# shubhamchandak94/Spring

Hardware: AMD Instinct MI355X
Metric: Mreads/s through reorder stage (higher is better)
Workload: dtype u64

## Files before the change

spring_amd/csrc/reorder_device.h:

```cpp
#ifndef SPRING_REORDER_DEVICE_H_
#define SPRING_REORDER_DEVICE_H_

#include <hip/hip_runtime.h>
#include <stdint.h>

namespace sr {

constexpr int MAX_READ_LEN = 511;
constexpr int MAX_SEARCH = 1000;
constexpr int THRESH = 4;
constexpr uint32_t DEEP_BIN = 16;
constexpr uint32_t MID_BIN = 64;
constexpr uint32_t BIG_BIN = 256;
constexpr uint32_t CHUNK = 64;
constexpr uint32_t MARK_BLOCK = 256;
constexpr uint32_t MC_WAVES_PER_BLOCK = MARK_BLOCK / 4 + 3;
constexpr int UBLK_SHIFT = 12;
constexpr int LDS_PAD = 10;
constexpr int LDS_LIMBS = 16 + 2 * LDS_PAD;

enum { MODE_SEARCH = 0, MODE_NEED_SEED = 1 };
enum { PROP_NONE = 0, PROP_MATCH = 1, PROP_SEED = 2, PROP_FRESH = 3  };
enum { PK_NONE = 0, PK_MATCH = 1, PK_SEED = 2, PK_NOSEED = 4, PK_DONE = 5 };
constexpr unsigned long long PK_CURSOR_BIT = 1ull << 35;
// ... 35 lines not shown
  uint64_t st_probes, st_keyok, st_cands, st_iter, st_lost, st_hits, n_unmatched, st_long ;
#ifdef SR_PHASE_TIMING
  uint64_t pt[64];
#endif
};
#ifndef SR_PHASE_TIMING
static_assert(sizeof(Chain) == 384, "Chain layout");
#endif

struct Globals {
  long long cursor;
  uint32_t alive;
  uint32_t e_alloc;
  uint32_t s_alloc;
  uint32_t pad;
  long long cursor_b;
};

struct TabView {
  const uint4 *buck;
  int bshift;
  int minz;
  int lshift;
};
constexpr uint32_t TAG_MARK = 0xfffffffcu;
constexpr int MINZ_HEAVY = 12;
constexpr int MINZ_K = 16;
constexpr int MINZ_WL = 32;

constexpr int LONG_MAX_BINS = 1024;
constexpr int LONG_MAX_PARTS = 64;
struct LongHead {
  uint32_t nb, nparts, best_single, bestrid;
  uint32_t bestpart, pad[3];
  uint32_t blo[LONG_MAX_PARTS + 4];
  uint32_t rescode[LONG_MAX_PARTS], resrid[LONG_MAX_PARTS];
  uint32_t capped[LONG_MAX_PARTS];
};
struct DevParams {
  const uint64_t *reads;
  const uint16_t *lens;
  uint32_t n;
  int L, W, S, Lpad, maxshift, uniform_len;
  int plan[2][6];
  int seed_wide;
  int deep_bins;
// ... 43 lines not shown
  unsigned long long *prop;
  uint32_t *alive_wave;
  Chain *chains;
  int4 *cnt;
  uint32_t *cnt8;
  uint4 *e_rec; uint2 *e_chunk;
  uint32_t *s_rec; uint2 *s_chunk;
  uint32_t *f_order; char *f_rc; char *f_flag; long long *f_pos; uint16_t *f_len; uint32_t *f_order_s;
};

void launch_unpack(hipStream_t st, const uint8_t *dna, const uint64_t *off, uint32_t n, int L, int W, int S,
                   uint32_t rec_fixed, uint64_t *reads, uint16_t *lens, uint32_t *bad_len = nullptr);
void launch_flag_in_dict(hipStream_t st, const uint16_t *lens, uint32_t n, int dend, uint32_t *flag);
void launch_keys(hipStream_t st, const uint64_t *reads, const uint16_t *lens, const uint32_t *slot, uint32_t n,
                 int S, int dstart, int dend, uint64_t *keys, uint32_t *vals);
struct DictBuild {
  const uint32_t *ustart, *ucount, *ids;
  ulonglong2 *urec;
  uint32_t *deep, *ndeep;
};
void launch_tab_insert(hipStream_t st, const uint64_t *mhash, const uint64_t *mval, uint64_t nmerged, DictBuild d0,
                       DictBuild d1, uint32_t *fpt, int bshift);
void launch_minz_prepare(hipStream_t st, const uint64_t *mhash, const uint64_t *mval, uint64_t nmerged, DictBuild d0,
                         DictBuild d1, int lshift, uint32_t *bucket, uint64_t *tagpay);
void launch_tab_insert_minz(hipStream_t st, const uint32_t *bucket_sorted, const uint64_t *tagpay_sorted, uint64_t nmerged,
                            uint32_t *fpt, int bshift, uint32_t *marked);
hipError_t sort_pairs_u32_u64(hipStream_t st, void *tmp, size_t &tmp_bytes, const uint32_t *kin, uint32_t *kout,
                              const uint64_t *vin, uint64_t *vout, size_t n, unsigned end_bit);
hipError_t merge_by_hash(hipStream_t st, void *tmp, size_t &tmp_bytes, const uint64_t *k0, const uint64_t *k1,
                         const uint64_t *v0, const uint64_t *v1, uint64_t *kout, uint64_t *vout, size_t n0, size_t n1);
void launch_iota_tag(hipStream_t st, uint64_t *v, uint64_t n, uint64_t tag);
void launch_build_epos(hipStream_t st, const uint32_t *ids, uint64_t m, uint32_t *epos);
void launch_trim_bins(hipStream_t st, const uint32_t *deep, const uint32_t *ndeep, uint32_t ndeep_host,
                      ulonglong2 *urec, const uint32_t *ids, const uint64_t *taken, ulonglong2 *sig ,
                      uint32_t *epos = nullptr );
void launch_build_sig(hipStream_t st, const uint32_t *ids, uint64_t m, const uint64_t *reads, int S, int W, ulonglong2 *sig);
void launch_dict_lookup(hipStream_t st, TabView tab, const ulonglong2 *urec, int which,
                        const uint64_t *reads, int S, int dstart, int dend, const uint64_t *keys, uint32_t nkeys,
                        uint32_t *start, uint32_t *count);
void launch_fill_u32(hipStream_t st, uint32_t *p, uint64_t n, uint32_t v);
void launch_init_taken(hipStream_t st, uint64_t *taken, uint64_t nwords, uint32_t n, uint32_t *ublk);
void launch_init_chains(hipStream_t st, const DevParams &P, bool seeds = true);
void launch_check_seed_state(hipStream_t st, const DevParams &P, uint64_t nwords, unsigned long long *bad);
void launch_search(hipStream_t st, const DevParams &P, bool stats);
void launch_apply(hipStream_t st, const DevParams &P, bool literal);
void launch_round(hipStream_t st, const DevParams &P, bool stats, bool mg);
void launch_mg_resolve(hipStream_t st, const DevParams &P);
void launch_mg_mark(hipStream_t st, const DevParams &P);
void launch_ph_mark(hipStream_t st, const DevParams &P);
// ... 33 lines not shown
```

spring_amd/csrc/reorder_kernels.hip:

```cpp
#include <cstdlib>
#include <cstring>
#include <hip/hip_runtime.h>
#include <rocprim/rocprim.hpp>

#include "reorder_device.h"
#include "synth_common.h"

namespace sr {


__device__ __forceinline__ uint64_t mix64(uint64_t x) {
  x ^= x >> 33; x *= 0xff51afd7ed558ccdull; x ^= x >> 33; x *= 0xc4ceb9fe1a85ec53ull; x ^= x >> 33;
  return x;
}

__device__ __forceinline__ void wave_sync() {
  __builtin_amdgcn_fence(__ATOMIC_SEQ_CST, "wavefront");
  __builtin_amdgcn_wave_barrier();
}

__device__ __forceinline__ int uni_i32(int v) { return __builtin_amdgcn_readfirstlane(v); }
template <class T>
__device__ __forceinline__ T *uni_ptr(T *p) {
  const uint64_t a = reinterpret_cast<uint64_t>(p);
// ... 55 lines not shown
  return f == 0u ? 1u : f == 0x3fffffffu ? 0x3ffffffeu : f;
}
__device__ __forceinline__ uint64_t bucket_of(uint64_t h, int bshift) { return h >> bshift; }
__device__ __forceinline__ uint64_t bucket_mask(int bshift) { return (1ull << (64 - bshift)) - 1; }
__device__ __forceinline__ uint64_t unmix64(uint64_t x) {
  x ^= x >> 33; x *= 0x9cb4b2f8129337dbull; x ^= x >> 33; x *= 0x4f74430c22a54005ull; x ^= x >> 33;
  return x;
}
__device__ __forceinline__ uint32_t fmix32(uint32_t x) {
  x ^= x >> 16; x *= 0x85ebca6bu; x ^= x >> 13; x *= 0xc2b2ae35u; x ^= x >> 16;
  return x;
}
__device__ __forceinline__ uint32_t kmer_order(uint32_t x) {
  uint32_t r = __builtin_bitreverse32(x);
  r = ~(((r >> 1) & 0x55555555u) | ((r & 0x55555555u) << 1));
  return ((x < r ? x : r) ^ 0x5bd1e995u) * 0x9e3779b1u;
}
__device__ __forceinline__ uint32_t minz_of_key(uint64_t key) {
  uint32_t m = 0xffffffffu;
#pragma unroll
  for (int q = 0; q <= MINZ_WL - MINZ_K; q++) m = min(m, kmer_order((uint32_t)(key >> (2 * q))));
  return fmix32(m);
}
__device__ __forceinline__ uint64_t tab_home(const TabView &T, uint64_t h, uint32_t mz) {
  return T.minz ? (((uint64_t)(mz >> T.lshift) << 2) | ((h >> 30) & 3ull)) : bucket_of(h, T.bshift);
}
__device__ __forceinline__ uint64_t tab_redirect_x(uint32_t x32, int bshift) { return mix64(0x6a09e667f3bcc908ull ^ x32) >> bshift; }
__device__ __forceinline__ uint64_t tab_redirect(const TabView &T, uint64_t h) {
  return tab_redirect_x(fp30_of(h) | ((uint32_t)((h >> 30) & 3ull) << 30), T.bshift);
}
template <bool MZ = false>
__device__ __forceinline__ int tab_find(const TabView &T, uint64_t h, uint32_t mz, int l, int skip,
                                        uint32_t &pay, bool &other) {
  const uint32_t mine = (fp30_of(h) << 2) | ((uint32_t)l << 1), theirs = mine ^ 2u;
  const uint64_t bmask = bucket_mask(T.bshift);
  uint64_t b = MZ ? tab_home(T, h, mz) : bucket_of(h, T.bshift);
  bool first = MZ && T.minz != 0;
  for (;;) {
#if defined(SR_TAGS_NT)
    typedef uint32_t u32x4_t __attribute__((ext_vector_type(4)));
    const u32x4_t tv = __builtin_nontemporal_load(reinterpret_cast<const u32x4_t *>(&T.buck[b * 2]));
    const uint4 t = make_uint4(tv.x, tv.y, tv.z, tv.w);
#elif defined(SR_TAGS_SC)
    typedef uint32_t u32x4_t __attribute__((ext_vector_type(4)));
    u32x4_t tv;
    asm volatile("global_load_dwordx4 %0, %1, off sc0 sc1\n\ts_waitcnt vmcnt(0)" : "=v"(tv) : "v"(&T.buck[b * 2]) : "memory");
    const uint4 t = make_uint4(tv.x, tv.y, tv.z, tv.w);
#else
    const uint4 t = T.buck[b * 2];
#endif
    if (MZ && first) {
      first = false;
      if (t.x == TAG_MARK) { b = tab_redirect(T, h); continue; }
    }
    other = other || (t.x & ~1u) == theirs || (t.y & ~1u) == theirs || (t.z & ~1u) == theirs || t.w != 0;
    uint32_t m = (uint32_t)((t.x & ~1u) == mine) | ((uint32_t)((t.y & ~1u) == mine) << 1) |
                 ((uint32_t)((t.z & ~1u) == mine) << 2) | ((uint32_t)((t.w & ~1u) == mine) << 3);
    const int c = __popc(m);
    if (c > skip) {
// ... 111 lines not shown
  if (cn >= BIG_BIN) atomicAdd(d.ndeep + 1, cn);
  if (cn >= MID_BIN) atomicAdd(d.ndeep + 2, cn);
  d.urec[u] = make_ulonglong2(unmix64(h), (uint64_t)st | ((uint64_t)cn << 32));
  if (!OVERFLOW) {
    fpt[b0 * 8 + rank] = tag;
    fpt[b0 * 8 + 4 + rank] = pay;
    return;
  }
  const uint64_t bmask = bucket_mask(bshift);
  uint64_t b = (b0 + 1) & bmask;
  for (;;) {
    uint32_t *bk = fpt + b * 8;
    for (int sl = 0; sl < 4; sl++) {
      if (atomicCAS(bk + sl, 0u, tag) == 0u) {
        bk[4 + sl] = pay;
        return;
      }
    }
    b = (b + 1) & bmask;
  }
}

__global__ void k_minz_prepare(const uint64_t *__restrict__ mhash, const uint64_t *__restrict__ mval, uint64_t nm,
                               DictBuild d0, DictBuild d1, int lshift, uint32_t *__restrict__ bucket,
                               uint64_t *__restrict__ tagpay) {
  const uint64_t i = (uint64_t)blockIdx.x * blockDim.x + threadIdx.x;
  if (i >= nm) return;
  const uint64_t h = mhash[i], key = unmix64(h);
  const uint64_t mv = mval[i];
  const uint32_t l = (uint32_t)(mv >> 63), u = (uint32_t)mv;
  const DictBuild &d = l ? d1 : d0;
  const uint32_t st = d.ustart[u], cn = d.ucount[u];
  const bool single = cn == 1;
  const uint32_t tag = (fp30_of(h) << 2) | (l << 1) | (single ? 1u : 0u);
  const uint32_t pay = single ? d.ids[st] : u;
  if (cn >= DEEP_BIN) d.deep[atomicAdd(d.ndeep, 1u)] = u;
  if (cn >= BIG_BIN) atomicAdd(d.ndeep + 1, cn);
  if (cn >= MID_BIN) atomicAdd(d.ndeep + 2, cn);
  d.urec[u] = make_ulonglong2(key, (uint64_t)st | ((uint64_t)cn << 32));
  bucket[i] = ((minz_of_key(key) >> lshift) << 2) | (uint32_t)((h >> 30) & 3ull);
  tagpay[i] = (uint64_t)tag | ((uint64_t)pay << 32);
}
template <bool SECOND>
__global__ void k_tab_insert_minz(const uint32_t *__restrict__ bk, const uint64_t *__restrict__ tp, uint64_t nm,
                                  uint32_t *fpt, int bshift, uint32_t *marked ) {
  const uint64_t i = (uint64_t)blockIdx.x * blockDim.x + threadIdx.x;
  if (i >= nm) return;
  const uint32_t b0 = bk[i], line = b0 >> 2;
  int back = 0;
  while (back <= MINZ_HEAVY && i > (uint64_t)back && (bk[i - 1 - back] >> 2) == line) back++;
  bool heavy = back > MINZ_HEAVY;
  if (!heavy) {
    const uint64_t at = i - back + MINZ_HEAVY;
    heavy = at < nm && (bk[at] >> 2) == line;
  }
  int rank = 0;
  if (!heavy) while (rank < 4 && rank < back && bk[i - 1 - rank] == b0) rank++;
  const uint64_t w = tp[i];
  const uint32_t tag = (uint32_t)w, pay = (uint32_t)(w >> 32);
  if (!SECOND) {
    if (heavy) {
      if (back == 0) {
        for (int s = 0; s < 4; s++) fpt[((uint64_t)line * 4 + s) * 8] = TAG_MARK;
        atomicAdd(marked, 1u);
      }
    } else if (rank < 4) {
      fpt[(uint64_t)b0 * 8 + rank] = tag;
      fpt[(uint64_t)b0 * 8 + 4 + rank] = pay;
    }
    return;
  }
  if (!heavy && rank < 4) return;
  const uint64_t bmask = bucket_mask(bshift);
  uint64_t b = heavy ? tab_redirect_x((tag >> 2) | ((b0 & 3u) << 30), bshift) : (((uint64_t)b0 + 1) & bmask);
  for (;;) {
// ... 33 lines not shown
    const uint32_t pos = w + (uint32_t)__popcll(m & ((1ull << lane) - 1));
    if (live && pos != j) {
      ids[start + pos] = r;
      if (sig) sig[start + pos] = sg;
      if (epos) epos[r] = start + pos;
    }
    w += (uint32_t)__popcll(m);
  }
  if (lane == 0 && w != count) urec[u].y = (uint64_t)start | ((uint64_t)w << 32);
}

__global__ void k_dict_lookup(TabView tab, const ulonglong2 *__restrict__ urec, int which,
                              const uint64_t *__restrict__ reads, int S, int dstart, int klen2,
                              const uint64_t *__restrict__ keys, uint32_t nkeys, uint32_t *__restrict__ start,
                              uint32_t *__restrict__ count) {
  uint32_t i = blockIdx.x * blockDim.x + threadIdx.x;
  if (i >= nkeys) return;
  const uint64_t key = keys[i], h = mix64(key);
  const uint32_t mz = tab.minz ? minz_of_key(key) : 0u;
  uint32_t s = 0, c = 0xffffffffu;
  for (int skip = 0;; skip++) {
    uint32_t pay;
    bool other = false;
    const int kind = tab_find<true>(tab, h, mz, which, skip, pay, other);
    if (kind == 0) break;
    if (kind == 1) {
      const ulonglong2 r = urec[pay];
      if (r.x != key) continue;
      s = (uint32_t)r.y; c = (uint32_t)(r.y >> 32);
      break;
    }
    if (read_window(reads + (uint64_t)pay * S, S, dstart, klen2) != key) continue;
    s = pay; c = 1u | 0x80000000u;
    break;
  }
  start[i] = s;
  count[i] = c;
}

__global__ void k_fill_u32(uint32_t *p, uint64_t n, uint32_t v) {
  uint64_t i = (uint64_t)blockIdx.x * blockDim.x + threadIdx.x;
  if (i < n) p[i] = v;
}

__global__ void k_init_taken(uint64_t *taken, uint64_t nwords, uint32_t n, uint32_t *ublk) {
  uint64_t w = (uint64_t)blockIdx.x * blockDim.x + threadIdx.x;
  if (w >= nwords) return;
// ... 508 lines not shown
                                           bool &keyok, uint32_t &ncand, bool &other, lds_u32_t *s_best, lds_u32_t *stage,
                                           int lane, PendBin *pend = nullptr, int *walk_left = nullptr, int pre = 0) {
  const int ds = l ? uni_i32(P.dstart[1]) : uni_i32(P.dstart[0]);
  const int klen2 = 2 * P.wl;
  typedef unsigned long long u64x2_t __attribute__((ext_vector_type(2)));
  typedef const __attribute__((address_space(1))) u64x2_t g_urec_t;
  typedef const __attribute__((address_space(1))) uint32_t g_u32_t;
  g_urec_t *urec = (g_urec_t *)(l ? uni_ptr(P.urec[1]) : uni_ptr(P.urec[0]));
  g_u32_t *ids = (g_u32_t *)(l ? uni_ptr(P.ids[1]) : uni_ptr(P.ids[0]));
  const int bitshift = rev ? -2 * shift : 2 * shift;
  const int lo = rev ? shift : 0;
  const int mref = rev ? ref_len + shift : ref_len - shift;
  auto within_thresh = [&](uint32_t r, bool check_key) -> int {
    return cmp_candidate<TRIM>(P, sx, bitshift, lo, mref, ds, klen2, r, check_key, stage, lane, SPEC ? P.taken : nullptr);
  };
  const uint32_t mycode = (uint32_t)((shift << 2) | (rev << 1) | l);
  auto beaten = [&]() -> bool { return *(volatile lds_u32_t *)s_best < mycode; };
  for (int skip = 0;; skip++) {
    if (skip && beaten()) break;
    uint32_t pay;
    int kind;
    if (MZ && skip == 0 && pre) {
      kind = pre & 3;
      pay = reinterpret_cast<const uint32_t *>(P.tab.buck)[tab_home(P.tab, hsh, mz) * 8 + 4 + (pre >> 2)];
    } else kind = tab_find<MZ>(P.tab, hsh, mz, l, skip, pay, other);
    if (skip == 0) PTW(12);
    if (kind == 0) break;
    const bool single = kind == 2;
    uint32_t start = 0, count = 1;
    if (!single) {
      const u64x2_t rec = urec[pay];
      if (rec.x != key) continue;
      start = (uint32_t)rec.y; count = (uint32_t)(rec.y >> 32);
      if (DEFER) { pend->on = true; pend->start = start; pend->count = count; pend->pay = pay; break; }
    }
    bool verified = !single, gave_up = false;
    int live = 0, top_live = -1;
    for (int j = (int)count - 1; j >= 0 && live < MAX_SEARCH; j--) {
      if (j != (int)count - 1 && beaten()) { gave_up = true; break; }
      if (walk_left && --(*walk_left) < 0) {
        if (j >= P.long_min >> 6) {
          __hip_atomic_fetch_min(s_best, 0u, __ATOMIC_RELAXED, __HIP_MEMORY_SCOPE_WAVEFRONT);
          gave_up = true;
          break;
        }
        *walk_left = j;
      }
      uint32_t r = single ? pay : ids[start + j];
// ... 17 lines not shown
    break;
  }
}

template <bool QUAD>
__device__ __forceinline__ uint32_t find_alt(const DevParams &P, const uint64_t *sref, const uint64_t *srev, int ref_len,
                                             int code, uint32_t wrid, lds_u32_t *stage, int lane) {
  const int l = code & 1, rev = (code >> 1) & 1, shift = code >> 2;
  const int ds = l ? uni_i32(P.dstart[1]) : uni_i32(P.dstart[0]);
  const int klen2 = 2 * P.wl;
  const uint64_t kmask = klen2 < 64 ? ((1ull << klen2) - 1) : ~0ull;
  const uint64_t *sx = rev ? srev : sref;
  const uint64_t key = lds_window(sx, rev ? 2 * (ds - shift) : 2 * (ds + shift)) & kmask;
  const uint64_t hsh = mix64(key);
  typedef unsigned long long u64x2_t __attribute__((ext_vector_type(2)));
  typedef const __attribute__((address_space(1))) u64x2_t g_urec_t;
  typedef const __attribute__((address_space(1))) uint32_t g_u32_t;
  g_urec_t *urec = (g_urec_t *)(l ? uni_ptr(P.urec[1]) : uni_ptr(P.urec[0]));
  g_u32_t *ids = (g_u32_t *)(l ? uni_ptr(P.ids[1]) : uni_ptr(P.ids[0]));
  uint32_t start = 0, count = 0;
  for (int skip = 0;; skip++) {
    uint32_t pay;
    bool other = false;
    const int kind = uni_i32(tab_find<false>(P.tab, hsh, 0u, l, skip, pay, other));
    if (kind == 0) return 0xffffffffu;
    if (kind == 2) { if (uni_u32(pay) == wrid) return 0xffffffffu; continue; }
    const u64x2_t rec = urec[uni_u32(pay)];
    if (rec.x != key) continue;
    start = uni_u32((uint32_t)rec.y); count = uni_u32((uint32_t)(rec.y >> 32));
    break;
  }
  const int bitshift = rev ? -2 * shift : 2 * shift;
  const int lo = rev ? shift : 0;
  const int mref = rev ? ref_len + shift : ref_len - shift;
  int livec = 0;
  bool seen = false;
  for (uint32_t base = 0; base < count; base += 64) {
    const long long j = (long long)count - 1 - ((long long)base + lane);
    uint32_t r = 0;
    bool live = false;
    if (j >= 0) {
      r = ids[start + (uint32_t)j];
      bool tr_;
      live = !entry_dead(P, r, tr_);
    }
    const uint64_t Lm = __ballot(live);
    uint64_t cand = Lm;
// ... 1594 lines not shown

#define GRID1(n, bs) dim3((unsigned)(((uint64_t)(n) + (bs) - 1) / (bs)))

void launch_unpack(hipStream_t st, const uint8_t *dna, const uint64_t *off, uint32_t n, int L, int W, int S,
                   uint32_t rec_fixed, uint64_t *reads, uint16_t *lens, uint32_t *bad_len) {
  if (!n) return;
  uint64_t tot = (uint64_t)n * S;
  hipLaunchKernelGGL(k_unpack, GRID1(tot, 256), dim3(256), 0, st, dna, off, n, L, W, S, rec_fixed, reads, lens, bad_len);
}
void launch_flag_in_dict(hipStream_t st, const uint16_t *lens, uint32_t n, int dend, uint32_t *flag) {
  hipLaunchKernelGGL(k_flag_in_dict, GRID1(n, 256), dim3(256), 0, st, lens, n, dend, flag);
}
void launch_keys(hipStream_t st, const uint64_t *reads, const uint16_t *lens, const uint32_t *slot, uint32_t n,
                 int S, int dstart, int dend, uint64_t *keys, uint32_t *vals) {
  hipLaunchKernelGGL(k_keys, GRID1(n, 256), dim3(256), 0, st, reads, lens, slot, n, S, dstart, dend, keys, vals);
}
void launch_tab_insert(hipStream_t st, const uint64_t *mhash, const uint64_t *mval, uint64_t nmerged, DictBuild d0,
                       DictBuild d1, uint32_t *fpt, int bshift) {
  if (!nmerged) return;
  hipLaunchKernelGGL(k_tab_insert<false>, GRID1(nmerged, 256), dim3(256), 0, st, mhash, mval, nmerged, d0, d1, fpt, bshift);
  hipLaunchKernelGGL(k_tab_insert<true>, GRID1(nmerged, 256), dim3(256), 0, st, mhash, mval, nmerged, d0, d1, fpt, bshift);
}
void launch_minz_prepare(hipStream_t st, const uint64_t *mhash, const uint64_t *mval, uint64_t nmerged, DictBuild d0,
                         DictBuild d1, int lshift, uint32_t *bucket, uint64_t *tagpay) {
  if (!nmerged) return;
  hipLaunchKernelGGL(k_minz_prepare, GRID1(nmerged, 256), dim3(256), 0, st, mhash, mval, nmerged, d0, d1, lshift, bucket, tagpay);
}
void launch_tab_insert_minz(hipStream_t st, const uint32_t *bucket_sorted, const uint64_t *tagpay_sorted, uint64_t nmerged,
                            uint32_t *fpt, int bshift, uint32_t *marked) {
  if (!nmerged) return;
  hipLaunchKernelGGL(k_tab_insert_minz<false>, GRID1(nmerged, 256), dim3(256), 0, st, bucket_sorted, tagpay_sorted, nmerged, fpt, bshift, marked);
  hipLaunchKernelGGL(k_tab_insert_minz<true>, GRID1(nmerged, 256), dim3(256), 0, st, bucket_sorted, tagpay_sorted, nmerged, fpt, bshift, marked);
}
void launch_iota_tag(hipStream_t st, uint64_t *v, uint64_t n, uint64_t tag) {
  if (!n) return;
  hipLaunchKernelGGL(k_iota_tag, GRID1(n, 256), dim3(256), 0, st, v, n, tag);
}
void launch_trim_bins(hipStream_t st, const uint32_t *deep, const uint32_t *ndeep, uint32_t ndeep_host,
                      ulonglong2 *urec, const uint32_t *ids, const uint64_t *taken, ulonglong2 *sig, uint32_t *epos) {
  if (!ndeep_host) return;
  hipLaunchKernelGGL(k_trim_bins, GRID1(ndeep_host, 4), dim3(256), 0, st, deep, ndeep, urec, const_cast<uint32_t *>(ids), taken, sig, epos);
}
void launch_dict_lookup(hipStream_t st, TabView tab, const ulonglong2 *urec, int which,
                        const uint64_t *reads, int S, int dstart, int dend, const uint64_t *keys, uint32_t nkeys,
                        uint32_t *start, uint32_t *count) {
  if (!nkeys) return;
  hipLaunchKernelGGL(k_dict_lookup, GRID1(nkeys, 256), dim3(256), 0, st, tab, urec, which, reads, S, dstart,
                     2 * (dend - dstart + 1), keys, nkeys, start, count);
}
void launch_fill_u32(hipStream_t st, uint32_t *p, uint64_t n, uint32_t v) {
  if (!n) return;
  hipLaunchKernelGGL(k_fill_u32, GRID1(n, 256), dim3(256), 0, st, p, n, v);
}
__global__ void k_check_seed_state(DevParams P, uint64_t nwords, unsigned long long *bad) {
  const uint64_t w = (uint64_t)blockIdx.x * blockDim.x + threadIdx.x;
// ... 181 lines not shown
```

spring_amd/csrc/reorder_pipeline.cpp:

```cpp
#include <hip/hip_runtime.h>
#include <dlfcn.h>

#include <algorithm>
#include <system_error>
#include <thread>
#include <memory>
#include <atomic>
#include <chrono>
#include <cstdarg>
#include <cstdio>
#include <cstdlib>
#include <cstring>
#include <map>
#include <mutex>
#include <new>
#include <stdexcept>
#include <string>
#include <unordered_map>
#include <vector>
#include <zlib.h>

#include "reorder_device.h"
#include "reorder_internal.h"
#include "spring_reorder.h"
// ... 82 lines not shown
  uint32_t mid_reads = 0;
};

struct spring_reorder_ctx {
  spring_reorder_opts o;
  int dev = 0;
  hipStream_t st = nullptr;
  int stage = ST_CREATED;
  std::vector<void *> allocs;
  uint64_t dev_bytes = 0, peak_bytes = 0;
  uint8_t *d_dna = nullptr;
  bool dna_borrowed = false;
  size_t dna_bytes = 0;
  uint64_t *d_off = nullptr;
  uint32_t n = 0;
  int L = 0, W = 0, S = 0, Lpad = 0;
  bool uniform = true;
  uint64_t *d_reads = nullptr;
  uint16_t *d_lens = nullptr;
  DictDev dict[2];
  uint4 *fpt = nullptr;
  int bshift = 63;
  int minz = 0, lshift = 31;
  uint32_t marked_lines = 0;
  bool user_plan0 = false;
  DevParams P;
  uint32_t K = 0;
  uint64_t nrec = 0, nsing = 0, cap = 0;
  bool mg = false;
  uint32_t *cnt_buf[2] = {nullptr, nullptr};
  uint64_t round_no = 0;
  hipStream_t st2 = nullptr, st3 = nullptr;
  uint64_t *taken2 = nullptr;
  uint32_t *resv2 = nullptr, *won = nullptr;
  uint32_t Kh = 0, nmid = 0;
  struct GroupGeom { uint32_t g0 = 0, Kg = 0, c0 = 0, gg0 = 0, gKg = 0; } grp[2];
  struct LongBufs { uint32_t *longq = nullptr, *lctl = nullptr, *lparts = nullptr; LongHead *lhead = nullptr; uint2 *lbin = nullptr; uint16_t *lbcode = nullptr; } lb2;
  bool in_source_fallback = false;
  uint8_t *d_N[2] = {nullptr, nullptr};
  uint32_t *d_orderN[2] = {nullptr, nullptr};
  uint64_t *d_offN[2] = {nullptr, nullptr};
  uint64_t N_bytes[2] = {0, 0};
  spring_fastq_info fq;
  double fq_ms = 0;
  std::vector<uint64_t> tid_off, tid_off_s;
  std::vector<uint64_t> tid_mid, tid_mid_s;
// ... 803 lines not shown
    HIPCHK(hipMemcpy2D(limbs, (size_t)ctx->W * 8, ctx->d_reads, (size_t)ctx->S * 8, (size_t)ctx->W * 8, ctx->n,
                       hipMemcpyDeviceToHost));
  if (len) HIPCHK(hipMemcpy(len, ctx->d_lens, (size_t)ctx->n * 2, hipMemcpyDeviceToHost));
  return 0;
}

static uint64_t pow2ceil(uint64_t x) {
  uint64_t p = 1;
  while (p < x) p <<= 1;
  return p;
}

static double now_ms() {
  return std::chrono::duration<double, std::milli>(std::chrono::steady_clock::now().time_since_epoch()).count();
}
#define DBG_T(label)                                                                         \
  do {                                                                                       \
    if (dbg) { (void)hipStreamSynchronize(st); double t_ = now_ms(); fprintf(stderr, "[dict] %-14s %8.2f ms\n", label, t_ - t_last); t_last = t_; } \
  } while (0)

static TabView tab_view(const spring_reorder_ctx *ctx) {
  TabView t;
  t.buck = ctx->fpt;
  t.bshift = ctx->bshift; t.minz = ctx->minz; t.lshift = ctx->lshift;
  return t;
}

int spring_reorder_build_dict(spring_reorder_ctx *ctx) {
  double t_last = now_ms();
  if (!ctx) return fail(SPRING_REORDER_E_ARG, "ctx is NULL");
  const bool dbg = ctx->o.debug != 0;
  if (ctx->stage != ST_LOADED) return fail(SPRING_REORDER_E_STATE, "build_dict: load reads first");
  HIPCHK(hipSetDevice(ctx->dev));
  hipStream_t st = ctx->st;
  const uint32_t n = ctx->n;
  HIPCHK(hipEventRecord(ctx->ev[2], st));
  uint64_t *uhash[2] = {nullptr, nullptr};
  uint32_t *ustart[2] = {nullptr, nullptr}, *ucount[2] = {nullptr, nullptr};
  for (int l = 0; l < 2; l++) {
    DictDev &d = ctx->dict[l];
    uint32_t m = 0;
    uint32_t *d_slot = nullptr, *d_flag = nullptr;
    void *d_tmp = nullptr;
    size_t tmp_bytes = 0;
    if (n) {
      if (ctx->uniform) {
        m = ctx->L > d.end ? n : 0;
// ... 59 lines not shown
    tmp_bytes = 0;
    HIPCHK(excl_scan_u32(st, nullptr, tmp_bytes, cnt, ustart[l], numkeys));
    DMALLOC(d_tmp, tmp_bytes);
    HIPCHK(excl_scan_u32(st, d_tmp, tmp_bytes, cnt, ustart[l], numkeys));
    DBG_T("scan");
    uhash[l] = k_in;
    ucount[l] = cnt;
    DMALLOC(d.urec, (size_t)numkeys * 16);
    DMALLOC(d.deep, ((size_t)m / DEEP_BIN + 1) * 4);
    DMALLOC(d.d_ndeep, 16);
    HIPCHK(hipMemsetAsync(d.d_ndeep, 0, 12, st));
    HIPCHK(hipStreamSynchronize(st));
    ctx->dfree(d_tmp);
    if (d_flag) { ctx->dfree(d_flag); ctx->dfree(d_slot); }
  }
  const uint64_t nk0 = ctx->dict[0].numkeys, nk1 = ctx->dict[1].numkeys, nm = nk0 + nk1;
  const int tab_scale = ctx->o.tab_scale > 0 ? ctx->o.tab_scale : 2;
  const uint64_t nb = std::max<uint64_t>(8, pow2ceil(std::max<uint64_t>(2, (nm * 10 + 15) / 16)) * (uint64_t)pow2ceil(tab_scale));
  ctx->bshift = 64;
  for (uint64_t v = nb; v > 1; v >>= 1) ctx->bshift--;
  ctx->minz = (ctx->dict[0].end - ctx->dict[0].start + 1 == MINZ_WL && ctx->L <= 192 && ctx->o.table_mode == 2) ? 1 : 0;
  ctx->lshift = 32 - (64 - ctx->bshift - 2);
  if (ctx->lshift < 1) return fail(SPRING_REORDER_E_ARG, "build_dict: table too large for minimizer addressing");
  ctx->stats.table_minz = ctx->minz; ctx->stats.table_marked_lines = 0;
  DMALLOC(ctx->fpt, nb * 32);
  HIPCHK(hipMemsetAsync(ctx->fpt, 0, nb * 32, st));
  uint32_t *const tab_words = reinterpret_cast<uint32_t *>(ctx->fpt);
  DBG_T("alloc+memset tab");
  if (nm) {
    uint64_t *mv0 = nullptr, *mv1 = nullptr, *mh = nullptr, *mv = nullptr;
    void *d_tmp = nullptr;
    DMALLOC(mv0, std::max<uint64_t>(nk0, 1) * 8);
    DMALLOC(mv1, std::max<uint64_t>(nk1, 1) * 8);
    launch_iota_tag(st, mv0, nk0, 0ull);
    launch_iota_tag(st, mv1, nk1, 1ull << 63);
    const uint64_t *h_in = nullptr, *v_in = nullptr;
    if (nk0 && nk1) {
      DMALLOC(mh, nm * 8);
      DMALLOC(mv, nm * 8);
      size_t tb = 0;
      HIPCHK(merge_by_hash(st, nullptr, tb, uhash[0], uhash[1], mv0, mv1, mh, mv, nk0, nk1));
      DMALLOC(d_tmp, tb);
      HIPCHK(merge_by_hash(st, d_tmp, tb, uhash[0], uhash[1], mv0, mv1, mh, mv, nk0, nk1));
      h_in = mh; v_in = mv;
    } else {
      h_in = nk0 ? uhash[0] : uhash[1];
      v_in = nk0 ? mv0 : mv1;
    }
    DBG_T("merge");
    DictBuild db[2];
    for (int l = 0; l < 2; l++) {
      DictDev &d = ctx->dict[l];
      db[l].ustart = ustart[l]; db[l].ucount = ucount[l]; db[l].ids = d.ids; db[l].urec = d.urec;
      db[l].deep = d.deep; db[l].ndeep = d.d_ndeep;
    }
    uint32_t *bk_in = nullptr, *bk_out = nullptr, *d_marked = nullptr;
    uint64_t *tp_in = nullptr, *tp_out = nullptr;
    ctx->marked_lines = 0;
    void *d_tmp2 = nullptr;
    if (!ctx->minz) {
      launch_tab_insert(st, h_in, v_in, nm, db[0], db[1], tab_words, ctx->bshift);
    } else {
      DMALLOC(bk_in, nm * 4); DMALLOC(bk_out, nm * 4);
      DMALLOC(tp_in, nm * 8); DMALLOC(tp_out, nm * 8);
      launch_minz_prepare(st, h_in, v_in, nm, db[0], db[1], ctx->lshift, bk_in, tp_in);
      DBG_T("minz prepare");
      const unsigned end_bit = (unsigned)(64 - ctx->bshift);
      size_t tb = 0;
      HIPCHK(sort_pairs_u32_u64(st, nullptr, tb, bk_in, bk_out, tp_in, tp_out, nm, end_bit));
      DMALLOC(d_tmp2, tb);
      HIPCHK(sort_pairs_u32_u64(st, d_tmp2, tb, bk_in, bk_out, tp_in, tp_out, nm, end_bit));
      DBG_T("minz sort");
      DMALLOC(d_marked, 16);
      HIPCHK(hipMemsetAsync(d_marked, 0, 4, st));
      launch_tab_insert_minz(st, bk_out, tp_out, nm, tab_words, ctx->bshift, d_marked);
      HIPCHK(hipMemcpyAsync(&ctx->marked_lines, d_marked, 4, hipMemcpyDeviceToHost, st));
    }
    HIPCHK(hipGetLastError());
    uint32_t nd[2][3] = {{0, 0, 0}, {0, 0, 0}};
    for (int l = 0; l < 2; l++)
      HIPCHK(hipMemcpyAsync(nd[l], ctx->dict[l].d_ndeep, 12, hipMemcpyDeviceToHost, st));
    HIPCHK(hipStreamSynchronize(st));
    for (int l = 0; l < 2; l++) { ctx->dict[l].ndeep = nd[l][0]; ctx->dict[l].big_reads = nd[l][1]; ctx->dict[l].mid_reads = nd[l][2]; }
    if (dbg) fprintf(stderr, "[dict] reads %u + %u, keys %u + %u, bins >= %u: %u + %u, reads in bins >= %u: %u + %u, >= %u: %u + %u\n",
                     ctx->dict[0].numreads, ctx->dict[1].numreads, ctx->dict[0].numkeys, ctx->dict[1].numkeys, DEEP_BIN, nd[0][0], nd[1][0],
                     MID_BIN, nd[0][2], nd[1][2], BIG_BIN, nd[0][1], nd[1][1]);
    ctx->stats.table_marked_lines = ctx->marked_lines;
    DBG_T("insert");
    ctx->dfree(mv0); ctx->dfree(mv1); ctx->dfree(mh); ctx->dfree(mv); ctx->dfree(d_tmp);
    ctx->dfree(bk_in); ctx->dfree(bk_out); ctx->dfree(tp_in); ctx->dfree(tp_out); ctx->dfree(d_tmp2); ctx->dfree(d_marked);
  }
  for (int l = 0; l < 2; l++) { ctx->dfree(uhash[l]); ctx->dfree(ustart[l]); ctx->dfree(ucount[l]); }
  DBG_T("free temps");
  HIPCHK(hipEventRecord(ctx->ev[3], st));
  ctx->stage = ST_DICT;
  return 0;
}

int spring_reorder_dict_lookup(spring_reorder_ctx *ctx, int32_t which, const uint64_t *keys, uint32_t nkeys,
                               uint32_t *bin_size, uint32_t *bin_ids, size_t ids_cap) {
  if (!ctx || ctx->stage < ST_DICT) return fail(SPRING_REORDER_E_STATE, "dict_lookup: build_dict first");
  if (which < 0 || which > 1) return fail(SPRING_REORDER_E_ARG, "which must be 0 or 1");
  HIPCHK(hipSetDevice(ctx->dev));
  DictDev &d = ctx->dict[which];
  uint64_t *dk = nullptr;
  uint32_t *ds = nullptr, *dc = nullptr;
  DMALLOC(dk, (size_t)nkeys * 8);
  DMALLOC(ds, (size_t)nkeys * 4);
  DMALLOC(dc, (size_t)nkeys * 4);
  std::vector<uint32_t> hs(nkeys), hc(nkeys), hids(d.numreads);
  if (nkeys) {
    HIPCHK(hipMemcpyAsync(dk, keys, (size_t)nkeys * 8, hipMemcpyHostToDevice, ctx->st));
    launch_dict_lookup(ctx->st, tab_view(ctx), d.urec, which, ctx->d_reads, ctx->S, d.start, d.end, dk, nkeys, ds, dc);
// ... 1314 lines not shown
```

spring_amd/csrc/reorder_round_mc.h:

```cpp
#ifndef SPRING_REORDER_ROUND_MC_H_
#define SPRING_REORDER_ROUND_MC_H_

namespace mc {

constexpr int G = 16;
constexpr int CPW = 64 / G;

template <int NQ, bool KA>
struct GLds {
  static constexpr int WMAX = NQ <= 3 ? 6 : 16;
  static constexpr int PAD = NQ <= 3 ? 4 : LDS_PAD;
  static constexpr int LIMBS = WMAX + 2 * PAD;
  static constexpr int MZ = NQ <= 3 && !KA ? 164 : 4;
  uint64_t refs[2][LIMBS];
  uint64_t rd[WMAX + 2];
  uint64_t nref[WMAX];
  union {
    uint8_t pres[128];
    uint64_t ka[2][KA ? LIMBS : 2];
  };
  uint32_t best;
  uint32_t pad[3];
  uint32_t mz[MZ];
};
// ... 465 lines not shown
  lds_u32_t *s_best = (lds_u32_t *)&S.best;
  if (gl == 0) *s_best = (uint32_t)INF_CODE;
  wave_sync();
  const uint32_t bmask = (uint32_t)bucket_mask(P.tab.bshift);
  uint4 tg[4];
  uint64_t key[4];
  uint32_t bk[4];
  bool val[4];
#pragma unroll
  for (int i = 0; i < 4; i++) {
    const int code = c_lo + gl + G * i;
    const int l = code & 1, rev = (code >> 1) & 1, shift = code >> 2;
    val[i] = code < c_hi && probe_valid(P, l, rev, shift, ref_len);
    key[i] = 0;
    bk[i] = 0;
    tg[i] = make_uint4(0, 0, 0, 0);
    if (val[i]) {
      const int ds = l ? P.dstart[1] : P.dstart[0];
      key[i] = lds_window(rev ? srev : sref, rev ? 2 * (ds - shift) : 2 * (ds + shift)) & kmask;
      const int o = rev ? ds - shift : ds + shift;
#ifdef SR_EXP_FAKE
      tg[i] = P.tab.buck[exp_fake_quad(P, sref, rev ? ref_len - P.wl - o : o, key[i])];
#else
      bk[i] = (uint32_t)tab_home(P.tab, mix64(key[i]), minz ? S.mz[rev ? ref_len - MINZ_WL - o : o] : 0u);
      tg[i] = P.tab.buck[2 * (uint64_t)bk[i]];
#endif
    }
  }
  PT(25);
  PTW(26);
  uint32_t pend = 0, cont = 0, redir = 0, oth = 0, pre = 0;
#pragma unroll
  for (int i = 0; i < 4; i++) {
    if (!val[i]) continue;
    const int code = c_lo + gl + G * i;
    if (minz && tg[i].x == TAG_MARK) { cont |= 1u << i; redir |= 1u << i; continue; }
    bool other = false;
    int slot = 0;
    const int st = tags_step(tg[i], mix64(key[i]), code & 1, other, slot);
    if (other) oth |= 1u << i;
    if (st == 1) { pend |= 1u << i; pre |= (uint32_t)((1 + ((slot >> 2) & 1)) | ((slot & 3) << 2)) << (4 * i); }
    else if (st == 2) cont |= 1u << i;
  }
  for (int hop = 0; hop < QUICK_HOPS && __ballot(cont != 0); hop++) {
#pragma unroll
    for (int i = 0; i < 4; i++)
      if ((cont >> i) & 1u) {
// ... 81 lines not shown
        i = rev ? idx - nF : idx;
        if (!rev) {
          const int sh0 = t0 + i, sh1 = sh0 - wl;
          v0 = probe_valid(P, 0, 0, sh0, ref_len);
          v1 = sh1 >= t0 && probe_valid(P, 1, 0, sh1, ref_len);
          if (v0 && sh1 >= 0 && sh1 < t0) v0 = S.pres[4 * sh1 + 1] != 0;
        } else {
          const int sh1 = t0 + i, sh0 = sh1 - wl;
          v1 = probe_valid(P, 1, 1, sh1, ref_len);
          v0 = sh0 >= t0 && probe_valid(P, 0, 1, sh0, ref_len);
          if (v1 && sh0 >= 0 && sh0 < t0) v1 = S.pres[4 * sh0 + 2] != 0;
        }
      }
      desc[k] = ((uint32_t)rev << 31) | ((uint32_t)v1 << 30) | ((uint32_t)v0 << 29) | (uint32_t)i;
      key[k] = 0;
      bk[k] = 0;
      tg[k] = make_uint4(0, 0, 0, 0);
      if (v0 || v1) {
        const int off = rev ? s1 - (t0 + i) : s0 + t0 + i;
        key[k] = lds_window(rev ? srev : sref, 2 * off) & kmask;
#ifdef SR_EXP_FAKE
        tg[k] = P.tab.buck[exp_fake_quad(P, sref, rev ? ref_len - wl - off : off, key[k])];
#else
        bk[k] = (uint32_t)tab_home(P.tab, mix64(key[k]), minz ? S.mz[rev ? ref_len - MINZ_WL - off : off] : 0u);
        tg[k] = P.tab.buck[2 * (uint64_t)bk[k]];
#endif
      }
    }
    PT(28);
    PTW(29);
    uint32_t pend = 0, un = 0, cont = 0, redir = 0, pre = 0;
#pragma unroll
    for (int k = 0; k < 4; k++) {
      const uint32_t e = desc[k];
      if (!(e & (3u << 29))) continue;
      const int rev = (int)(e >> 31);
#pragma unroll
      for (int j = 0; j < 2; j++) {
        const int l = rev ? j : 1 - j;
        if ((e >> (29 + l)) & 1u) un |= 1u << (2 * k + j);
      }
      if (minz && tg[k].x == TAG_MARK) { cont |= 1u << k; redir |= 1u << k; continue; }
      const uint64_t hsh = mix64(key[k]);
#pragma unroll
      for (int j = 0; j < 2; j++) {
        if (!((un >> (2 * k + j)) & 1u)) continue;
        const int l = rev ? j : 1 - j;
// ... 146 lines not shown
  const int wl = P.wl, klen2 = 2 * wl;
  const uint64_t kmask = klen2 < 64 ? ((1ull << klen2) - 1) : ~0ull;
  lds_u32_t *s_best = (lds_u32_t *)&S.best;
  const uint32_t bmask = (uint32_t)bucket_mask(P.tab.bshift);
  uint4 tg[KA_M];
  uint64_t key[KA_M];
  uint32_t bk[KA_M];
  int code[KA_M];
#pragma unroll
  for (int i = 0; i < KA_M; i++) {
    code[i] = -1;
    key[i] = 0;
    bk[i] = 0;
    tg[i] = make_uint4(0, 0, 0, 0);
    if (i < m && need) {
      const int b = __ffs((int)need) - 1;
      need &= need - 1;
      const int cd = ka_code_of_bit(b, gl, wl);
      code[i] = cd;
      const int l = cd & 1, rev = (cd >> 1) & 1, shift = cd >> 2;
      const int ds = l ? P.dstart[1] : P.dstart[0];
      const int o = rev ? ds - shift : ds + shift;
      key[i] = lds_window(rev ? srev : sref, 2 * o) & kmask;
      bk[i] = (uint32_t)bucket_of(mix64(key[i]), P.tab.bshift);
      tg[i] = P.tab.buck[2 * (uint64_t)bk[i]];
    }
  }
  uint32_t pend = 0, cont = 0, oth = 0, pre = 0;
#pragma unroll
  for (int i = 0; i < KA_M; i++) {
    if (code[i] < 0) continue;
    bool other = false;
    int slot = 0;
    const int st = tags_step(tg[i], mix64(key[i]), code[i] & 1, other, slot);
    if (other) oth |= 1u << i;
    if (st == 1) { pend |= 1u << i; pre |= (uint32_t)((1 + ((slot >> 2) & 1)) | ((slot & 3) << 2)) << (4 * i); }
    else if (st == 2) cont |= 1u << i;
  }
  for (int hop = 0; hop < QUICK_HOPS && __ballot(cont != 0); hop++) {
#pragma unroll
    for (int i = 0; i < KA_M; i++)
      if ((cont >> i) & 1u) {
        bk[i] = (bk[i] + 1u) & bmask;
        tg[i] = P.tab.buck[2 * (uint64_t)bk[i]];
      }
    const uint32_t c2 = cont;
    cont = 0;
#pragma unroll
    for (int i = 0; i < KA_M; i++)
      if ((c2 >> i) & 1u) {
        bool other = false;
        int slot = 0;
        const int st = tags_step(tg[i], mix64(key[i]), code[i] & 1, other, slot);
        if (other) oth |= 1u << i;
        if (st == 1) pend |= 1u << i;
        else if (st == 2) cont |= 1u << i;
      }
  }
  pend |= cont;
  oth |= cont;
#pragma unroll
  for (int i = 0; i < KA_M; i++) {
    if (code[i] < 0) continue;
    const int cd = code[i], l = cd & 1, rev = (cd >> 1) & 1, shift = cd >> 2;
    const uint32_t own = ((pend >> i) & 1u) ^ 1u, other = ((oth >> i) & 1u) ^ 1u;
    const uint32_t bits = (own << l) | (other << (1 - l));
    if (bits) {
      const int ds = l ? P.dstart[1] : P.dstart[0];
      const int o = rev ? ds - shift : ds + shift;
      lds_u32_t *w = (lds_u32_t *)(S.ka[rev] + LDS_PAD) + (o >> 4);
      __hip_atomic_fetch_or(w, bits << (2 * (o & 15)), __ATOMIC_RELAXED, __HIP_MEMORY_SCOPE_WAVEFRONT);
    }
  }
  while (__ballot(pend != 0)) {
    if (pend) {
      const int i = __ffs((int)pend) - 1;
      pend &= pend - 1;
      int cd = code[0];
#pragma unroll
      for (int q = 1; q < KA_M; q++) cd = i == q ? code[q] : cd;
      const int l = cd & 1, rev = (cd >> 1) & 1, shift = cd >> 2;
      if (cd < best && !(*(volatile lds_u32_t *)s_best < (uint32_t)cd)) {
        bool hit = false, keyok = false, other = false;
        uint32_t rid = 0, ncand = 0;
        const int ds = l ? P.dstart[1] : P.dstart[0], o = rev ? ds - shift : ds + shift;
        const uint64_t k = lds_window(rev ? srev : sref, 2 * o) & kmask;
        eval_probe<false, false, false, true>(P, rev ? srev : sref, l, rev, shift, ref_len, k, mix64(k),
                                       0u, hit, rid, keyok, ncand, other, s_best, stage,
                                       lane, nullptr, nullptr, (int)((pre >> (4 * i)) & 15u));
        if (hit) { best = cd; brid = rid; }
      }
    }
  }
}
// ... 201 lines not shown
```

Baseline: 322.2.

## Place k-mers at a canonical home bucket so one probe rules out the reverse complement

When table_mode is 0 and both dictionaries share a window length of at most 32, the hash table places each k-mer in the bucket of its canonical (min of forward and reverse-complement) hash. The table build sorts entries by that bucket and reuses the existing sorted-insert path. During the quick search, a bucket that is not full and lacks the reverse-complement fingerprint lets the kernel mark the mirrored window on the opposite strand as known-absent, so that probe is skipped. The change also frees build temporaries early and reuses the value buffer for payloads to lower peak memory. In exchange it adds reverse-complement computation per probe and changes the table layout, so occupancy and collision chains shift.

Measured after the change: 336.9, median of 6. +4.6%, better.

```diff
diff --git a/spring_amd/csrc/reorder_device.h b/spring_amd/csrc/reorder_device.h
--- a/spring_amd/csrc/reorder_device.h
+++ b/spring_amd/csrc/reorder_device.h
@@ -81,6 +81,7 @@
   int bshift;
   int minz;
   int lshift;
+  int cwl;
 };
 constexpr uint32_t TAG_MARK = 0xfffffffcu;
 constexpr int MINZ_HEAVY = 12;
@@ -170,9 +171,9 @@
 void launch_tab_insert(hipStream_t st, const uint64_t *mhash, const uint64_t *mval, uint64_t nmerged, DictBuild d0,
                        DictBuild d1, uint32_t *fpt, int bshift);
 void launch_minz_prepare(hipStream_t st, const uint64_t *mhash, const uint64_t *mval, uint64_t nmerged, DictBuild d0,
-                         DictBuild d1, int lshift, uint32_t *bucket, uint64_t *tagpay);
+                         DictBuild d1, int lshift, int cwl, int bshift, uint32_t *bucket, uint64_t *tagpay);
 void launch_tab_insert_minz(hipStream_t st, const uint32_t *bucket_sorted, const uint64_t *tagpay_sorted, uint64_t nmerged,
-                            uint32_t *fpt, int bshift, uint32_t *marked);
+                            uint32_t *fpt, int bshift, uint32_t *marked, int minz);
 hipError_t sort_pairs_u32_u64(hipStream_t st, void *tmp, size_t &tmp_bytes, const uint32_t *kin, uint32_t *kout,
                               const uint64_t *vin, uint64_t *vout, size_t n, unsigned end_bit);
 hipError_t merge_by_hash(hipStream_t st, void *tmp, size_t &tmp_bytes, const uint64_t *k0, const uint64_t *k1,
diff --git a/spring_amd/csrc/reorder_kernels.hip b/spring_amd/csrc/reorder_kernels.hip
--- a/spring_amd/csrc/reorder_kernels.hip
+++ b/spring_amd/csrc/reorder_kernels.hip
@@ -101,19 +101,30 @@
   for (int q = 0; q <= MINZ_WL - MINZ_K; q++) m = min(m, kmer_order((uint32_t)(key >> (2 * q))));
   return fmix32(m);
 }
-__device__ __forceinline__ uint64_t tab_home(const TabView &T, uint64_t h, uint32_t mz) {
-  return T.minz ? (((uint64_t)(mz >> T.lshift) << 2) | ((h >> 30) & 3ull)) : bucket_of(h, T.bshift);
+__device__ __forceinline__ uint64_t rc_key(uint64_t k, int wl) {
+  uint32_t a = __builtin_bitreverse32((uint32_t)k), b = __builtin_bitreverse32((uint32_t)(k >> 32));
+  a = ~(((a >> 1) & 0x55555555u) | ((a & 0x55555555u) << 1));
+  b = ~(((b >> 1) & 0x55555555u) | ((b & 0x55555555u) << 1));
+  return (((uint64_t)a << 32) | b) >> (64 - 2 * wl);
+}
+__device__ __forceinline__ uint64_t home_hash(const TabView &T, uint64_t key, uint64_t h) {
+  if (!T.cwl) return h;
+  const uint64_t r = rc_key(key, T.cwl);
+  return mix64(r < key ? r : key);
+}
+__device__ __forceinline__ uint64_t tab_home(const TabView &T, uint64_t key, uint64_t h, uint32_t mz) {
+  return T.minz ? (((uint64_t)(mz >> T.lshift) << 2) | ((h >> 30) & 3ull)) : bucket_of(home_hash(T, key, h), T.bshift);
 }
 __device__ __forceinline__ uint64_t tab_redirect_x(uint32_t x32, int bshift) { return mix64(0x6a09e667f3bcc908ull ^ x32) >> bshift; }
 __device__ __forceinline__ uint64_t tab_redirect(const TabView &T, uint64_t h) {
   return tab_redirect_x(fp30_of(h) | ((uint32_t)((h >> 30) & 3ull) << 30), T.bshift);
 }
 template <bool MZ = false>
-__device__ __forceinline__ int tab_find(const TabView &T, uint64_t h, uint32_t mz, int l, int skip,
+__device__ __forceinline__ int tab_find(const TabView &T, uint64_t key, uint64_t h, uint32_t mz, int l, int skip,
                                         uint32_t &pay, bool &other) {
   const uint32_t mine = (fp30_of(h) << 2) | ((uint32_t)l << 1), theirs = mine ^ 2u;
   const uint64_t bmask = bucket_mask(T.bshift);
-  uint64_t b = MZ ? tab_home(T, h, mz) : bucket_of(h, T.bshift);
+  uint64_t b = MZ ? tab_home(T, key, h, mz) : bucket_of(home_hash(T, key, h), T.bshift);
   bool first = MZ && T.minz != 0;
   for (;;) {
 #if defined(SR_TAGS_NT)
@@ -271,7 +282,7 @@
 }
 
 __global__ void k_minz_prepare(const uint64_t *__restrict__ mhash, const uint64_t *__restrict__ mval, uint64_t nm,
-                               DictBuild d0, DictBuild d1, int lshift, uint32_t *__restrict__ bucket,
+                               DictBuild d0, DictBuild d1, int lshift, int cwl, int bshift, uint32_t *__restrict__ bucket,
                                uint64_t *__restrict__ tagpay) {
   const uint64_t i = (uint64_t)blockIdx.x * blockDim.x + threadIdx.x;
   if (i >= nm) return;
@@ -287,19 +298,23 @@
   if (cn >= BIG_BIN) atomicAdd(d.ndeep + 1, cn);
   if (cn >= MID_BIN) atomicAdd(d.ndeep + 2, cn);
   d.urec[u] = make_ulonglong2(key, (uint64_t)st | ((uint64_t)cn << 32));
-  bucket[i] = ((minz_of_key(key) >> lshift) << 2) | (uint32_t)((h >> 30) & 3ull);
+  if (cwl > 0) {
+    const uint64_t r = rc_key(key, cwl);
+    bucket[i] = (uint32_t)bucket_of(r < key ? mix64(r) : h, bshift);
+  } else bucket[i] = ((minz_of_key(key) >> lshift) << 2) | (uint32_t)((h >> 30) & 3ull);
   tagpay[i] = (uint64_t)tag | ((uint64_t)pay << 32);
 }
-template <bool SECOND>
+template <bool SECOND, bool MINZ>
 __global__ void k_tab_insert_minz(const uint32_t *__restrict__ bk, const uint64_t *__restrict__ tp, uint64_t nm,
                                   uint32_t *fpt, int bshift, uint32_t *marked ) {
   const uint64_t i = (uint64_t)blockIdx.x * blockDim.x + threadIdx.x;
   if (i >= nm) return;
-  const uint32_t b0 = bk[i], line = b0 >> 2;
+  const uint32_t b0 = bk[i], line = MINZ ? b0 >> 2 : b0;
   int back = 0;
-  while (back <= MINZ_HEAVY && i > (uint64_t)back && (bk[i - 1 - back] >> 2) == line) back++;
-  bool heavy = back > MINZ_HEAVY;
-  if (!heavy) {
+  const int bl = MINZ ? MINZ_HEAVY : 3;
+  while (back <= bl && i > (uint64_t)back && (MINZ ? bk[i - 1 - back] >> 2 : bk[i - 1 - back]) == line) back++;
+  bool heavy = MINZ && back > MINZ_HEAVY;
+  if (MINZ && !heavy) {
     const uint64_t at = i - back + MINZ_HEAVY;
     heavy = at < nm && (bk[at] >> 2) == line;
   }
@@ -379,7 +394,7 @@
   for (int skip = 0;; skip++) {
     uint32_t pay;
     bool other = false;
-    const int kind = tab_find<true>(tab, h, mz, which, skip, pay, other);
+    const int kind = tab_find<true>(tab, key, h, mz, which, skip, pay, other);
     if (kind == 0) break;
     if (kind == 1) {
       const ulonglong2 r = urec[pay];
@@ -934,8 +949,8 @@
     int kind;
     if (MZ && skip == 0 && pre) {
       kind = pre & 3;
-      pay = reinterpret_cast<const uint32_t *>(P.tab.buck)[tab_home(P.tab, hsh, mz) * 8 + 4 + (pre >> 2)];
-    } else kind = tab_find<MZ>(P.tab, hsh, mz, l, skip, pay, other);
+      pay = reinterpret_cast<const uint32_t *>(P.tab.buck)[tab_home(P.tab, key, hsh, mz) * 8 + 4 + (pre >> 2)];
+    } else kind = tab_find<MZ>(P.tab, key, hsh, mz, l, skip, pay, other);
     if (skip == 0) PTW(12);
     if (kind == 0) break;
     const bool single = kind == 2;
@@ -999,7 +1014,7 @@
   for (int skip = 0;; skip++) {
     uint32_t pay;
     bool other = false;
-    const int kind = uni_i32(tab_find<false>(P.tab, hsh, 0u, l, skip, pay, other));
+    const int kind = uni_i32(tab_find<false>(P.tab, key, hsh, 0u, l, skip, pay, other));
     if (kind == 0) return 0xffffffffu;
     if (kind == 2) { if (uni_u32(pay) == wrid) return 0xffffffffu; continue; }
     const u64x2_t rec = urec[uni_u32(pay)];
@@ -2640,15 +2655,20 @@
   hipLaunchKernelGGL(k_tab_insert<true>, GRID1(nmerged, 256), dim3(256), 0, st, mhash, mval, nmerged, d0, d1, fpt, bshift);
 }
 void launch_minz_prepare(hipStream_t st, const uint64_t *mhash, const uint64_t *mval, uint64_t nmerged, DictBuild d0,
-                         DictBuild d1, int lshift, uint32_t *bucket, uint64_t *tagpay) {
+                         DictBuild d1, int lshift, int cwl, int bshift, uint32_t *bucket, uint64_t *tagpay) {
   if (!nmerged) return;
-  hipLaunchKernelGGL(k_minz_prepare, GRID1(nmerged, 256), dim3(256), 0, st, mhash, mval, nmerged, d0, d1, lshift, bucket, tagpay);
+  hipLaunchKernelGGL(k_minz_prepare, GRID1(nmerged, 256), dim3(256), 0, st, mhash, mval, nmerged, d0, d1, lshift, cwl, bshift, bucket, tagpay);
 }
 void launch_tab_insert_minz(hipStream_t st, const uint32_t *bucket_sorted, const uint64_t *tagpay_sorted, uint64_t nmerged,
-                            uint32_t *fpt, int bshift, uint32_t *marked) {
+                            uint32_t *fpt, int bshift, uint32_t *marked, int minz) {
   if (!nmerged) return;
-  hipLaunchKernelGGL(k_tab_insert_minz<false>, GRID1(nmerged, 256), dim3(256), 0, st, bucket_sorted, tagpay_sorted, nmerged, fpt, bshift, marked);
-  hipLaunchKernelGGL(k_tab_insert_minz<true>, GRID1(nmerged, 256), dim3(256), 0, st, bucket_sorted, tagpay_sorted, nmerged, fpt, bshift, marked);
+  if (minz) {
+    hipLaunchKernelGGL((k_tab_insert_minz<false, true>), GRID1(nmerged, 256), dim3(256), 0, st, bucket_sorted, tagpay_sorted, nmerged, fpt, bshift, marked);
+    hipLaunchKernelGGL((k_tab_insert_minz<true, true>), GRID1(nmerged, 256), dim3(256), 0, st, bucket_sorted, tagpay_sorted, nmerged, fpt, bshift, marked);
+  } else {
+    hipLaunchKernelGGL((k_tab_insert_minz<false, false>), GRID1(nmerged, 256), dim3(256), 0, st, bucket_sorted, tagpay_sorted, nmerged, fpt, bshift, marked);
+    hipLaunchKernelGGL((k_tab_insert_minz<true, false>), GRID1(nmerged, 256), dim3(256), 0, st, bucket_sorted, tagpay_sorted, nmerged, fpt, bshift, marked);
+  }
 }
 void launch_iota_tag(hipStream_t st, uint64_t *v, uint64_t n, uint64_t tag) {
   if (!n) return;
diff --git a/spring_amd/csrc/reorder_pipeline.cpp b/spring_amd/csrc/reorder_pipeline.cpp
--- a/spring_amd/csrc/reorder_pipeline.cpp
+++ b/spring_amd/csrc/reorder_pipeline.cpp
@@ -128,6 +128,7 @@
   uint4 *fpt = nullptr;
   int bshift = 63;
   int minz = 0, lshift = 31;
+  int cwl = 0;
   uint32_t marked_lines = 0;
   bool user_plan0 = false;
   DevParams P;
@@ -977,7 +978,7 @@
 static TabView tab_view(const spring_reorder_ctx *ctx) {
   TabView t;
   t.buck = ctx->fpt;
-  t.bshift = ctx->bshift; t.minz = ctx->minz; t.lshift = ctx->lshift;
+  t.bshift = ctx->bshift; t.minz = ctx->minz; t.lshift = ctx->lshift; t.cwl = ctx->cwl;
   return t;
 }
 
@@ -1083,6 +1084,8 @@
   ctx->minz = (ctx->dict[0].end - ctx->dict[0].start + 1 == MINZ_WL && ctx->L <= 192 && ctx->o.table_mode == 2) ? 1 : 0;
   ctx->lshift = 32 - (64 - ctx->bshift - 2);
   if (ctx->lshift < 1) return fail(SPRING_REORDER_E_ARG, "build_dict: table too large for minimizer addressing");
+  const int wl0 = ctx->dict[0].end - ctx->dict[0].start + 1, wl1 = ctx->dict[1].end - ctx->dict[1].start + 1;
+  ctx->cwl = (!ctx->minz && ctx->o.table_mode == 0 && wl0 == wl1 && wl0 >= 1 && wl0 <= 32 && 64 - ctx->bshift <= 32) ? wl0 : 0;
   ctx->stats.table_minz = ctx->minz; ctx->stats.table_marked_lines = 0;
   DMALLOC(ctx->fpt, nb * 32);
   HIPCHK(hipMemsetAsync(ctx->fpt, 0, nb * 32, st));
@@ -1119,13 +1122,19 @@
     uint64_t *tp_in = nullptr, *tp_out = nullptr;
     ctx->marked_lines = 0;
     void *d_tmp2 = nullptr;
-    if (!ctx->minz) {
+    if (!ctx->minz && !ctx->cwl) {
       launch_tab_insert(st, h_in, v_in, nm, db[0], db[1], tab_words, ctx->bshift);
     } else {
-      DMALLOC(bk_in, nm * 4); DMALLOC(bk_out, nm * 4);
-      DMALLOC(tp_in, nm * 8); DMALLOC(tp_out, nm * 8);
-      launch_minz_prepare(st, h_in, v_in, nm, db[0], db[1], ctx->lshift, bk_in, tp_in);
+      DMALLOC(bk_in, nm * 4);
+      uint64_t *const tp_buf = const_cast<uint64_t *>(v_in);
+      launch_minz_prepare(st, h_in, v_in, nm, db[0], db[1], ctx->lshift, ctx->cwl, ctx->bshift, bk_in, tp_buf);
       DBG_T("minz prepare");
+      ctx->dfree(mh); mh = nullptr;
+      ctx->dfree(d_tmp); d_tmp = nullptr;
+      for (int l = 0; l < 2; l++) { ctx->dfree(uhash[l]); uhash[l] = nullptr; }
+      if (mv) { ctx->dfree(mv0); mv0 = nullptr; ctx->dfree(mv1); mv1 = nullptr; }
+      DMALLOC(bk_out, nm * 4); DMALLOC(tp_out, nm * 8);
+      tp_in = tp_buf;
       const unsigned end_bit = (unsigned)(64 - ctx->bshift);
       size_t tb = 0;
       HIPCHK(sort_pairs_u32_u64(st, nullptr, tb, bk_in, bk_out, tp_in, tp_out, nm, end_bit));
@@ -1134,7 +1143,7 @@
       DBG_T("minz sort");
       DMALLOC(d_marked, 16);
       HIPCHK(hipMemsetAsync(d_marked, 0, 4, st));
-      launch_tab_insert_minz(st, bk_out, tp_out, nm, tab_words, ctx->bshift, d_marked);
+      launch_tab_insert_minz(st, bk_out, tp_out, nm, tab_words, ctx->bshift, d_marked, ctx->minz);
       HIPCHK(hipMemcpyAsync(&ctx->marked_lines, d_marked, 4, hipMemcpyDeviceToHost, st));
     }
     HIPCHK(hipGetLastError());
@@ -1149,7 +1158,7 @@
     ctx->stats.table_marked_lines = ctx->marked_lines;
     DBG_T("insert");
     ctx->dfree(mv0); ctx->dfree(mv1); ctx->dfree(mh); ctx->dfree(mv); ctx->dfree(d_tmp);
-    ctx->dfree(bk_in); ctx->dfree(bk_out); ctx->dfree(tp_in); ctx->dfree(tp_out); ctx->dfree(d_tmp2); ctx->dfree(d_marked);
+    ctx->dfree(bk_in); ctx->dfree(bk_out); ctx->dfree(tp_out); ctx->dfree(d_tmp2); ctx->dfree(d_marked);
   }
   for (int l = 0; l < 2; l++) { ctx->dfree(uhash[l]); ctx->dfree(ustart[l]); ctx->dfree(ucount[l]); }
   DBG_T("free temps");
diff --git a/spring_amd/csrc/reorder_round_mc.h b/spring_amd/csrc/reorder_round_mc.h
--- a/spring_amd/csrc/reorder_round_mc.h
+++ b/spring_amd/csrc/reorder_round_mc.h
@@ -511,7 +511,7 @@
 #ifdef SR_EXP_FAKE
       tg[i] = P.tab.buck[exp_fake_quad(P, sref, rev ? ref_len - P.wl - o : o, key[i])];
 #else
-      bk[i] = (uint32_t)tab_home(P.tab, mix64(key[i]), minz ? S.mz[rev ? ref_len - MINZ_WL - o : o] : 0u);
+      bk[i] = (uint32_t)tab_home(P.tab, key[i], mix64(key[i]), minz ? S.mz[rev ? ref_len - MINZ_WL - o : o] : 0u);
       tg[i] = P.tab.buck[2 * (uint64_t)bk[i]];
 #endif
     }
@@ -639,7 +639,7 @@
 #ifdef SR_EXP_FAKE
         tg[k] = P.tab.buck[exp_fake_quad(P, sref, rev ? ref_len - wl - off : off, key[k])];
 #else
-        bk[k] = (uint32_t)tab_home(P.tab, mix64(key[k]), minz ? S.mz[rev ? ref_len - MINZ_WL - off : off] : 0u);
+        bk[k] = (uint32_t)tab_home(P.tab, key[k], mix64(key[k]), minz ? S.mz[rev ? ref_len - MINZ_WL - off : off] : 0u);
         tg[k] = P.tab.buck[2 * (uint64_t)bk[k]];
 #endif
       }
@@ -832,14 +832,21 @@
       const int ds = l ? P.dstart[1] : P.dstart[0];
       const int o = rev ? ds - shift : ds + shift;
       key[i] = lds_window(rev ? srev : sref, 2 * o) & kmask;
-      bk[i] = (uint32_t)bucket_of(mix64(key[i]), P.tab.bshift);
+      bk[i] = (uint32_t)bucket_of(home_hash(P.tab, key[i], mix64(key[i])), P.tab.bshift);
       tg[i] = P.tab.buck[2 * (uint64_t)bk[i]];
     }
   }
-  uint32_t pend = 0, cont = 0, oth = 0, pre = 0;
+  uint32_t pend = 0, cont = 0, oth = 0, pre = 0, mir = 0;
 #pragma unroll
   for (int i = 0; i < KA_M; i++) {
     if (code[i] < 0) continue;
+    if (P.tab.cwl && tg[i].w == 0) {
+      const uint32_t mf = fp30_of(mix64(rc_key(key[i], wl))) << 2;
+      const uint4 t = tg[i];
+      const uint32_t s0 = (uint32_t)((t.x & ~1u) == mf) | (uint32_t)((t.y & ~1u) == mf) | (uint32_t)((t.z & ~1u) == mf);
+      const uint32_t s1 = (uint32_t)((t.x & ~1u) == (mf | 2u)) | (uint32_t)((t.y & ~1u) == (mf | 2u)) | (uint32_t)((t.z & ~1u) == (mf | 2u));
+      mir |= ((s0 ^ 1u) | ((s1 ^ 1u) << 1)) << (2 * i);
+    }
     bool other = false;
     int slot = 0;
     const int st = tags_step(tg[i], mix64(key[i]), code[i] & 1, other, slot);
@@ -875,11 +882,17 @@
     const int cd = code[i], l = cd & 1, rev = (cd >> 1) & 1, shift = cd >> 2;
     const uint32_t own = ((pend >> i) & 1u) ^ 1u, other = ((oth >> i) & 1u) ^ 1u;
     const uint32_t bits = (own << l) | (other << (1 - l));
+    const int ds = l ? P.dstart[1] : P.dstart[0];
+    const int o = rev ? ds - shift : ds + shift;
     if (bits) {
-      const int ds = l ? P.dstart[1] : P.dstart[0];
-      const int o = rev ? ds - shift : ds + shift;
       lds_u32_t *w = (lds_u32_t *)(S.ka[rev] + LDS_PAD) + (o >> 4);
       __hip_atomic_fetch_or(w, bits << (2 * (o & 15)), __ATOMIC_RELAXED, __HIP_MEMORY_SCOPE_WAVEFRONT);
+    }
+    const uint32_t mbits = (mir >> (2 * i)) & 3u;
+    if (mbits) {
+      const int om = ref_len - wl - o;
+      lds_u32_t *w = (lds_u32_t *)(S.ka[rev ^ 1] + LDS_PAD) + (om >> 4);
+      __hip_atomic_fetch_or(w, mbits << (2 * (om & 15)), __ATOMIC_RELAXED, __HIP_MEMORY_SCOPE_WAVEFRONT);
     }
   }
   while (__ballot(pend != 0)) {
```
